# rasoolims/ImageTranslate

Hardware: AMD Instinct MI355X
Metric: train tokens/sec (whole node), 6L enc-dec d=512 seq128 b64, 1/2/4/8 GPU (higher is better)
Workload: dtype bf16; 1 GPU; 6L/6L enc-dec d=512 h=8 ff=2048 V=30000, src[64,128] tgt[64,128], synthetic random-token MT; global_batch=64, seq_len=128, parallelism=dp1, distinct_batches=8, directions=2

## Files before the change

imagetranslate_amd/csrc/gemm_ln.hip:

```cpp
#include "mma.hpp"

namespace {

constexpr int LN_BM = 32, LN_THREADS = 512, LN_RB = 128;
constexpr int LN_A_TILE = LN_BM * LN_RB;

struct GemmLnP {
  const void* A; int64_t lda; int64_t a_bytes;
  const void* W; int64_t ldw; int64_t w_bytes;
  const void* bias; const void* resid; int64_t ldr;
  const void* gamma; const void* beta;
  void* pre_ln; void* out; int64_t ldo;
  float* mean; float* rstd;
  int M, K, rotate, has_bias, has_resid;
  float eps, inv_keep; uint32_t drop_thresh; uint64_t seed;
  unsigned long long* trace;
};

template <int N> IMT_DEVICE void wait_vmcnt() { asm volatile("s_waitcnt vmcnt(%0)" ::"n"(N) : "memory"); }

template <typename T, int NTW, int SPLIT> struct LnDma {
  static constexpr int NTS = NTW / SPLIT;
  static constexpr int WP = 2 * NTS;
  __amdgpu_buffer_rsrc_t ra, rw;
  int voff_w[WP], voff_a, hstep;
  IMT_DEVICE void init(const GemmLnP& p, int m0, int wave) {
    constexpr int ES = sizeof(T);
    ra = __builtin_amdgcn_make_buffer_rsrc(const_cast<void*>(p.A), 0, (int)p.a_bytes, 0x00020000);
    rw = __builtin_amdgcn_make_buffer_rsrc(const_cast<void*>(p.W), 0, (int)p.w_bytes, 0x00020000);
    const int lane = threadIdx.x & 63, prow = lane >> 3, pc = lane & 7;
#pragma unroll
    for (int i = 0; i < WP; ++i) {
      const int lr = wave * 16 * NTS + 8 * i + prow;
      const int n = wave * 16 * NTW + 8 * i + prow;
      voff_w[i] = (int)(((int64_t)n * p.ldw) * ES + ((pc ^ swz<LN_RB>(lr)) << 4));
    }
    hstep = (int)((int64_t)16 * NTS * p.ldw * ES);
    voff_a = 0;
    if (wave < 4) {
      const int row = 8 * wave + prow;
      voff_a = (int)(((int64_t)(m0 + row) * p.lda) * ES + ((pc ^ swz<LN_RB>(row)) << 4));
    }
  }
  IMT_DEVICE void issue(char* st, int kt, int h, int wave) const {
    const int adv = kt * LN_RB;
    if (wave < 4)
      __builtin_amdgcn_raw_ptr_buffer_load_lds(ra, (__attribute__((address_space(3))) void*)(st + wave * 1024), 16, voff_a + adv, 0, 0, 0);
    const int wadv = adv + h * hstep;
#pragma unroll
    for (int i = 0; i < WP; ++i)
      __builtin_amdgcn_raw_ptr_buffer_load_lds(rw, (__attribute__((address_space(3))) void*)(st + LN_A_TILE + (wave * WP + i) * 1024), 16,
                                               voff_w[i] + wadv, 0, 0, 0);
  }
};

template <typename T, int NTW, int SPLIT, int NST>
__global__ __launch_bounds__(LN_THREADS) void gemm_ln_kernel(GemmLnP p) {
  constexpr int N = 128 * NTW, NTS = NTW / SPLIT, WP = 2 * NTS;
  constexpr int SLOT = LN_A_TILE + (N / SPLIT) * LN_RB;
  constexpr int ES = sizeof(T);
  typedef typename Frag<T>::type frag_t;
  typedef typename Vec4<T>::type raw_t;
  extern __shared__ __attribute__((aligned(16))) char smem[];
  float* red = reinterpret_cast<float*>(smem + NST * SLOT);

  const int nblk = (p.M + LN_BM - 1) / LN_BM;
  const int m0 = imt_xcd_block(blockIdx.x, nblk) * LN_BM;
  const int wave = __builtin_amdgcn_readfirstlane(threadIdx.x >> 6);
  const int lane = threadIdx.x & 63, r = lane & 15, g = lane >> 4;
  const int wn = wave * 16 * NTW;
  const int nt = (int)((int64_t)p.K * ES / LN_RB);
  const int ns = nt * SPLIT;

  LnDma<T, NTW, SPLIT> dma;
  dma.init(p, m0, wave);
  const int phase = p.rotate ? (int)((blockIdx.x >> 3) % (unsigned)nt) : 0;
  auto issue = [&](int q) {
    const int k = q / SPLIT + phase;
    dma.issue(smem + (q % NST) * SLOT, k >= nt ? k - nt : k, q % SPLIT, wave);
  };

  const T* bias = reinterpret_cast<const T*>(p.bias);
  const T* resid = reinterpret_cast<const T*>(p.resid);
  const T* gamma = reinterpret_cast<const T*>(p.gamma);
  const T* beta = reinterpret_cast<const T*>(p.beta);
  raw_t rres[2][NTW], rb[NTW], rg[NTW], rbe[NTW];
#pragma unroll
  for (int j = 0; j < NTW; ++j) {
    const int n = wn + 16 * j + 4 * g;
    rb[j] = Vec4<T>::load_raw(bias + n);
    rg[j] = Vec4<T>::load_raw(gamma + n);
    rbe[j] = Vec4<T>::load_raw(beta + n);
#pragma unroll
    for (int i = 0; i < 2; ++i) {
      const int64_t m = min(m0 + 16 * i + r, p.M - 1);
      rres[i][j] = Vec4<T>::load_raw(resid + m * p.ldr + n);
    }
  }

  f32x4 acc[2][NTW];
#pragma unroll
  for (int i = 0; i < 2; ++i)
#pragma unroll
    for (int j = 0; j < NTW; ++j) acc[i][j] = f32x4{0.f, 0.f, 0.f, 0.f};

#pragma unroll
  for (int s0 = 0; s0 < NST - 1; ++s0)
    if (s0 < ns) issue(s0);
  IMT_STAMP(p.trace, 0);
  for (int q0 = 0; q0 < ns; q0 += SPLIT) {
#pragma unroll
    for (int h = 0; h < SPLIT; ++h) {
      const int q = q0 + h;
      const int newer = min(NST - 2, ns - 1 - q);
      if (wave < 4) {
        if (newer >= 2) wait_vmcnt<2 * (WP + 1)>(); else if (newer == 1) wait_vmcnt<WP + 1>(); else wait_vmcnt<0>();
      } else {
        if (newer >= 2) wait_vmcnt<2 * WP>(); else if (newer == 1) wait_vmcnt<WP>(); else wait_vmcnt<0>();
      }
      asm volatile("s_barrier" ::: "memory");
      if (q == 0) IMT_STAMP(p.trace, 1);
      if (q + NST - 1 < ns) issue(q + NST - 1);
      const char* ta = smem + (q % NST) * SLOT;
      const char* tb = ta + LN_A_TILE;
#pragma unroll
      for (int ks = 0; ks < 2; ++ks) {
        frag_t fa[2], fb[NTS];
#pragma unroll
        for (int i = 0; i < 2; ++i) fa[i] = lds_frag_kcontig<T, LN_RB>(ta, 16 * i, 4 * ks);
#pragma unroll
        for (int j = 0; j < NTS; ++j) fb[j] = lds_frag_kcontig<T, LN_RB>(tb, wave * 16 * NTS + 16 * j, 4 * ks);
#pragma unroll
        for (int i = 0; i < 2; ++i)
#pragma unroll
          for (int j = 0; j < NTS; ++j) mma16(acc[i][h * NTS + j], fb[j], fa[i]);
      }
    }
  }
  IMT_STAMP(p.trace, 2);

  float s[2] = {0.f, 0.f};
#pragma unroll
  for (int i = 0; i < 2; ++i) {
    const int64_t m = m0 + 16 * i + r;
#pragma unroll
    for (int j = 0; j < NTW; ++j) {
      const int n = wn + 16 * j + 4 * g;
      f32x4 v = acc[i][j];
      if (p.has_bias) v += Vec4<T>::cvt(rb[j]);
      if (p.drop_thresh) dropout_apply4(v, p.seed, (uint64_t)m * (uint64_t)N + (uint64_t)n, p.drop_thresh, p.inv_keep);
      if (p.has_resid) v += Vec4<T>::cvt(rres[i][j]);
#pragma unroll
      for (int e = 0; e < 4; ++e) {
        v[e] = to_f32<T>(from_f32<T>(v[e]));
        s[i] += v[e];
      }
      acc[i][j] = v;
    }
  }
#pragma unroll
  for (int i = 0; i < 2; ++i) {
    s[i] += __shfl_xor(s[i], 16, 64);
    s[i] += __shfl_xor(s[i], 32, 64);
    if (g == 0) red[wave * 32 + 16 * i + r] = s[i];
  }
  __syncthreads();
  float mean[2], rstd[2], q[2] = {0.f, 0.f};
#pragma unroll
  for (int i = 0; i < 2; ++i) {
    float t = 0.f;
#pragma unroll
    for (int w = 0; w < 8; ++w) t += red[w * 32 + 16 * i + r];
    mean[i] = t / (float)N;
#pragma unroll
    for (int j = 0; j < NTW; ++j)
#pragma unroll
      for (int e = 0; e < 4; ++e) { const float d = acc[i][j][e] - mean[i]; q[i] += d * d; }
    q[i] += __shfl_xor(q[i], 16, 64);
    q[i] += __shfl_xor(q[i], 32, 64);
    if (g == 0) red[256 + wave * 32 + 16 * i + r] = q[i];
  }
  __syncthreads();
  IMT_STAMP(p.trace, 3);
  T* pre = reinterpret_cast<T*>(p.pre_ln);
  T* out = reinterpret_cast<T*>(p.out);
#pragma unroll
  for (int i = 0; i < 2; ++i) {
    float t = 0.f;
#pragma unroll
    for (int w = 0; w < 8; ++w) t += red[256 + w * 32 + 16 * i + r];
    rstd[i] = 1.0f / sqrtf(t / (float)N + p.eps);
    const int64_t m = m0 + 16 * i + r;
    if (m < p.M) {
#pragma unroll
      for (int j = 0; j < NTW; ++j) {
        const int n = wn + 16 * j + 4 * g;
        const f32x4 gv = Vec4<T>::cvt(rg[j]), bv = Vec4<T>::cvt(rbe[j]);
        f32x4 y;
#pragma unroll
        for (int e = 0; e < 4; ++e) y[e] = (acc[i][j][e] - mean[i]) * rstd[i] * gv[e] + bv[e];
        if (pre) Vec4<T>::store(pre + m * p.ldo + n, acc[i][j]);
        Vec4<T>::store(out + m * p.ldo + n, y);
      }
      if (wave == 0 && g == 0) {
        if (p.mean) p.mean[m] = mean[i];
        if (p.rstd) p.rstd[m] = rstd[i];
      }
    }
  }
  IMT_STAMP(p.trace, 4);
}

template <typename T, int NTW, int SPLIT, int NST>
int launch_gemm_ln(const GemmLnP& p, hipStream_t st) {
  constexpr int N = 128 * NTW;
  constexpr int LDS = NST * (LN_A_TILE + (N / SPLIT) * LN_RB) + 2 * 8 * 32 * 4;
  static_assert(LDS <= 160 * 1024, "ring does not fit the CU's LDS");
  auto k = gemm_ln_kernel<T, NTW, SPLIT, NST>;
  static bool attr = false;
  if (!attr) { (void)hipFuncSetAttribute(reinterpret_cast<const void*>(k), hipFuncAttributeMaxDynamicSharedMemorySize, LDS); attr = true; }
  const char* kind = sizeof(T) == 2 ? "gemm_ln_bf16" : "gemm_ln_f32";
  if (imt_prof_enabled() && getenv("IMT_PROF_SHAPES")) kind = imt_prof_intern(kind, p.M, N, p.K);
  ImtProfScope prof(kind, 2.0 * p.M * N * p.K, ((double)p.M * p.K + (double)N * p.K + 3.0 * p.M * N) * sizeof(T), st);
  const int blocks = imt_cdiv(p.M, LN_BM);
  ImtTrace tr("gemm_ln", blocks, st);
  GemmLnP pt = p;
  pt.trace = tr.dev;
  hipLaunchKernelGGL(k, dim3(blocks), dim3(LN_THREADS), LDS, st, pt);
  if (tr.dev) fprintf(stderr, "[gemm_ln %s %dx%dx%d]\n", kind, p.M, N, p.K);
  IMT_CHECK_LAUNCH();
  return IMT_OK;
}

}

extern "C" int imt_gemm_bias_residual_ln_supported(int dtype, int N, int K) {
  const int es = imt_dtype_bytes(dtype);
  return imt_ok_dtype(dtype) && N >= 128 && N <= 512 && N % 128 == 0 && K > 0 && ((int64_t)K * es) % LN_RB == 0;
}

extern "C" int imt_gemm_bias_residual_ln(int dtype, const void* x, int64_t ldx, const void* w, int64_t ldw, const void* bias,
                                         const void* resid, int64_t ldr, const void* gamma, const void* beta, void* pre_ln,
                                         void* out, int64_t ldo, float* mean, float* rstd, int M, int N, int K, float eps,
                                         float dropout_p, uint64_t dropout_seed, void* stream) {
  IMT_CHECK_ARG(imt_ok_dtype(dtype), "gemm_bias_residual_ln: bad dtype");
  IMT_CHECK_ARG(imt_gemm_bias_residual_ln_supported(dtype, N, K), "gemm_bias_residual_ln: N must be 128, 256, 384 or 512 and K a whole number of 128-byte tiles (N=%d K=%d)", N, K);
  if (M <= 0) return IMT_OK;
  const int es = imt_dtype_bytes(dtype), al = 16 / es;
  IMT_CHECK_ARG(x && w && gamma && beta && out, "gemm_bias_residual_ln: null pointer");
  IMT_CHECK_ARG(ldx % al == 0 && ldw % al == 0 && ldo % 4 == 0 && (!resid || ldr % 4 == 0), "gemm_bias_residual_ln: leading dimensions must keep rows 16-byte aligned");
  IMT_CHECK_ARG((((uintptr_t)x | (uintptr_t)w) & 15) == 0, "gemm_bias_residual_ln: x / w must be 16-byte aligned");
  IMT_CHECK_ARG(dropout_p >= 0.f && dropout_p < 1.f, "gemm_bias_residual_ln: dropout_p outside [0, 1)");
  GemmLnP p;
  p.A = x; p.lda = ldx; p.a_bytes = ((int64_t)(M - 1) * ldx + K) * es;
  p.W = w; p.ldw = ldw; p.w_bytes = ((int64_t)(N - 1) * ldw + K) * es;
  IMT_CHECK_ARG(p.a_bytes < (1ll << 31) && p.w_bytes < (1ll << 31), "gemm_bias_residual_ln: operand too large for 32-bit offsets");
  p.bias = bias ? bias : gamma; p.resid = resid ? resid : gamma; p.ldr = resid ? ldr : 0; p.gamma = gamma; p.beta = beta;
  p.has_bias = bias != nullptr; p.has_resid = resid != nullptr;
  p.pre_ln = pre_ln; p.out = out; p.ldo = ldo; p.mean = mean; p.rstd = rstd;
  p.M = M; p.K = K; p.eps = eps;
  static const bool no_rotate = getenv("IMT_GEMM_LN_NO_ROTATE") != nullptr;
  p.rotate = no_rotate ? 0 : 1;
  p.drop_thresh = dropout_thresh(dropout_p);
  p.inv_keep = dropout_p > 0.f ? 1.0f / (1.0f - dropout_p) : 1.0f;
  p.seed = dropout_seed;
  p.trace = nullptr;
  hipStream_t st = (hipStream_t)stream;
#define IMT_GLN(T)                                            \
  switch (N / 128) {                                          \
    case 1: return launch_gemm_ln<T, 1, 1, 4>(p, st);         \
    case 2: return launch_gemm_ln<T, 2, 1, 4>(p, st);         \
    case 3: return launch_gemm_ln<T, 3, 1, 3>(p, st);         \
    default: return launch_gemm_ln<T, 4, 2, 4>(p, st);        \
  }
  if (dtype == IMT_F32) { IMT_GLN(float) }
  IMT_GLN(bf16_t)
#undef IMT_GLN
}
```

imagetranslate_amd/csrc/model.hip:

```cpp
#include "common.hpp"
#include "decode_fused.hpp"

namespace {

struct Carver {
  char* base; int64_t off;
  explicit Carver(void* b) : base(reinterpret_cast<char*>(b)), off(0) {}
  void* take(int64_t bytes) {
    void* p = base ? base + off : nullptr;
    off += (bytes + 255) & ~(int64_t)255;
    return p;
  }
};

struct AttnWs {
  void* qkv;
  void* kv;
  int64_t kv_ld;
  void* ctx;
  float* lse;
  void* pre_ln;
  float* mean; float* rstd;
  void* out;
};
struct LayerWs {
  AttnWs self_attn, cross;
  void* z; void* h;
  void* pre_ln2; float* mean2; float* rstd2;
  void* out;
};
struct StackWs {
  void* emb_sum; float* emb_mean; float* emb_rstd; void* x0;
  LayerWs* layers;
  void* d_run;
  void* dpre[3]; void* ddrop[3];
  void* d_ctx;
  void* d_ff;
  void* d_qkv;
  void* d_q;
  void* d_kv;
  void* d_emb;
  struct Scratch { void* dpre[3]; void* ddrop[3]; void* d_ctx; void* d_ff; void* d_qkv; void* d_q; void* d_kv; } scr[2];
  void use_scratch(int l) {
    const Scratch& z = scr[l & 1];
    for (int i = 0; i < 3; ++i) { dpre[i] = z.dpre[i]; ddrop[i] = z.ddrop[i]; }
    d_ctx = z.d_ctx; d_ff = z.d_ff; d_qkv = z.d_qkv; d_q = z.d_q; d_kv = z.d_kv;
  }
  void* kv_all; void* d_kv_all;
  float* delta;
  float* ln_partial;
  float* ln_site(int site, int d) const { return ln_partial + (int64_t)site * IMT_LN_BWD_WS_FLOATS(d); }
  void* splitk; int64_t splitk_bytes;
  int64_t bytes;
};

constexpr int MAX_LAYERS = 64;

int64_t kv_w_off(const imt_stack_desc* m, const imt_layer_desc& p) { return p.cross_kv_w >= 0 ? p.cross_kv_w : p.cross_attn.qkv_w + (int64_t)m->d * m->d; }
int64_t kv_b_off(const imt_stack_desc* m, const imt_layer_desc& p) { return p.cross_kv_b >= 0 ? p.cross_kv_b : p.cross_attn.qkv_b + m->d; }
bool cross_kv_batched(const imt_stack_desc* m) {
  if (!m->is_decoder || m->n_layers < 2) return false;
  const int64_t d = m->d;
  for (int l = 0; l < m->n_layers; ++l) {
    const imt_layer_desc& p = m->layers[l];
    if (p.cross_attn.qkv_w < 0 || p.cross_kv_w < 0 || p.cross_kv_b < 0) return false;
    if (p.cross_kv_w != m->layers[0].cross_kv_w + (int64_t)l * 2 * d * d) return false;
    if (p.cross_kv_b != m->layers[0].cross_kv_b + (int64_t)l * 2 * d) return false;
  }
  return true;
}

void carve(const imt_stack_desc* m, int B, int T, int Tk, void* ws, StackWs& w, LayerWs* layers) {
  Carver c(ws);
  const int64_t N = (int64_t)B * T, Nk = (int64_t)B * Tk, d = m->d, ff = m->ff, es = imt_dtype_bytes(m->dtype);
  w.emb_sum = c.take(N * d * es); w.emb_mean = (float*)c.take(N * 4); w.emb_rstd = (float*)c.take(N * 4);
  w.x0 = c.take(N * d * es);
  w.layers = layers;
  const bool batched = cross_kv_batched(m);
  const int64_t L2d = (int64_t)m->n_layers * 2 * d;
  w.kv_all = w.d_kv_all = nullptr;
  if (batched) { w.kv_all = c.take(Nk * L2d * es); w.d_kv_all = c.take(Nk * L2d * es); }
  for (int l = 0; l < m->n_layers; ++l) {
    LayerWs& L = layers[l];
    AttnWs& s = L.self_attn;
    s.qkv = c.take(N * 3 * d * es); s.kv = nullptr; s.ctx = c.take(N * d * es);
    s.lse = (float*)c.take((int64_t)B * m->heads * T * 4);
    s.pre_ln = c.take(N * d * es); s.mean = (float*)c.take(N * 4); s.rstd = (float*)c.take(N * 4);
    s.out = c.take(N * d * es);
    AttnWs& x = L.cross;
    memset(&x, 0, sizeof(x));
    if (m->is_decoder && m->layers[l].cross_attn.qkv_w >= 0) {
      x.qkv = c.take(N * d * es); x.ctx = c.take(N * d * es);
      if (batched) { x.kv = w.kv_all ? (void*)((char*)w.kv_all + (int64_t)l * 2 * d * es) : nullptr; x.kv_ld = L2d; }
      else { x.kv = c.take(Nk * 2 * d * es); x.kv_ld = 2 * d; }
      x.lse = (float*)c.take((int64_t)B * m->heads * T * 4);
      x.pre_ln = c.take(N * d * es); x.mean = (float*)c.take(N * 4); x.rstd = (float*)c.take(N * 4);
      x.out = c.take(N * d * es);
    }
    L.z = c.take(N * ff * es); L.h = c.take(N * ff * es);
    L.pre_ln2 = c.take(N * d * es); L.mean2 = (float*)c.take(N * 4); L.rstd2 = (float*)c.take(N * 4);
    L.out = c.take(N * d * es);
  }
  w.d_run = c.take(N * d * es);
  for (int k = 0; k < 2; ++k) {
    StackWs::Scratch& z = w.scr[k];
    for (int i = 0; i < 3; ++i) { z.dpre[i] = c.take(N * d * es); z.ddrop[i] = c.take(N * d * es); }
    z.d_ctx = c.take(N * d * es);
    z.d_ff = c.take(N * ff * es);
    z.d_qkv = c.take(N * 3 * d * es);
    z.d_q = c.take(N * d * es);
    z.d_kv = c.take((Nk > 0 ? Nk : 1) * 2 * d * es);
  }
  w.use_scratch(0);
  w.d_emb = c.take(N * d * es);
  w.delta = (float*)c.take((int64_t)B * m->heads * T * 4);
  w.ln_partial = (float*)c.take((int64_t)(3 * m->n_layers + 1) * IMT_LN_BWD_WS_FLOATS(d) * 4);
  w.splitk_bytes = ((N + 127) / 128) * ((d + 127) / 128) <= 128 ? imt_gemm_splitk_ws_bytes() : 0;
  w.splitk = w.splitk_bytes ? c.take(w.splitk_bytes) : nullptr;
  w.bytes = c.off;
}

struct Ctx {
  const imt_stack_desc* m; hipStream_t st; int dtype; int64_t es;
  void* splitk = nullptr; int64_t splitk_bytes = 0;
  const char* P(int64_t off) const { return reinterpret_cast<const char*>(m->params) + off * es; }
  float* G(int64_t off) const { return m->grads + off; }
};

#define RC(x) do { int rc__ = (x); if (rc__ != IMT_OK) return rc__; } while (0)

int linear_fwd(const Ctx& c, const void* x, int64_t ldx, int M, int K, int64_t w_off, int64_t b_off, int N, void* y, int64_t ldy,
               const void* resid, int64_t ldr, void* aux, int aux_mode, float drop_p, uint64_t seed) {
  imt_gemm_args a;
  memset(&a, 0, sizeof(a));
  a.dtype = c.dtype; a.layout = IMT_NT; a.M = M; a.N = N; a.K = K;
  a.A = x; a.lda = ldx; a.B = c.P(w_off); a.ldb = K; a.C = y; a.ldc = ldy; a.c_dtype = c.dtype;
  a.bias = b_off >= 0 ? c.P(b_off) : nullptr;
  a.resid = resid; a.ldr = ldr; a.aux = aux; a.ldaux = N; a.aux_mode = aux_mode; a.split_k = 1; a.alpha = 1.f;
  a.dropout_p = drop_p; a.dropout_seed = seed;
  a.splitk_ws = c.splitk; a.splitk_ws_bytes = c.splitk_bytes;
  return imt_gemm(&a, c.st);
}

int linear_bwd_input(const Ctx& c, const void* dy, int64_t lddy, int M, int N, int64_t w_off, int K, void* dx, int64_t lddx,
                     const void* resid, int64_t ldr, void* aux, int aux_mode, int accumulate) {
  imt_gemm_args a;
  memset(&a, 0, sizeof(a));
  a.dtype = c.dtype; a.layout = IMT_NN; a.M = M; a.N = K; a.K = N;
  a.A = dy; a.lda = lddy; a.B = c.P(w_off); a.ldb = K; a.C = dx; a.ldc = lddx; a.c_dtype = c.dtype;
  a.resid = resid; a.ldr = ldr; a.aux = aux; a.ldaux = K; a.aux_mode = aux_mode; a.split_k = 1; a.alpha = 1.f;
  a.accumulate = accumulate;
  a.splitk_ws = c.splitk; a.splitk_ws_bytes = c.splitk_bytes;
  return imt_gemm(&a, c.st);
}

bool fuse_dense_ln(const Ctx& c, int M, int N, int K) {
  static const int mode = getenv("IMT_GEMM_LN") ? atoi(getenv("IMT_GEMM_LN")) : -1;
  if (mode == 0 || !imt_gemm_bias_residual_ln_supported(c.dtype, N, K)) return false;
  if (mode == 1) return true;
  return N <= 256 && K <= 1024;
}
int dense_resid_ln(const Ctx& c, const void* x, int64_t ldx, int M, int K, int64_t w_off, int64_t b_off, int N, const void* resid,
                   int64_t g_off, int64_t beta_off, void* pre_ln, void* out, float* mean, float* rstd, float drop_p, uint64_t seed) {
  if (fuse_dense_ln(c, M, N, K))
    return imt_gemm_bias_residual_ln(c.dtype, x, ldx, c.P(w_off), K, b_off >= 0 ? c.P(b_off) : nullptr, resid, N, c.P(g_off), c.P(beta_off),
                                     pre_ln, out, N, mean, rstd, M, N, K, c.m->ln_eps, drop_p, seed, c.st);
  imt_gemm_args a;
  memset(&a, 0, sizeof(a));
  a.dtype = c.dtype; a.layout = IMT_NT; a.M = M; a.N = N; a.K = K;
  a.A = x; a.lda = ldx; a.B = c.P(w_off); a.ldb = K; a.C = pre_ln; a.ldc = N; a.c_dtype = c.dtype;
  a.bias = b_off >= 0 ? c.P(b_off) : nullptr;
  a.resid = resid; a.ldr = N; a.aux_mode = IMT_AUX_NONE; a.split_k = 1; a.alpha = 1.f;
  a.dropout_p = drop_p; a.dropout_seed = seed;
  a.ln_gamma = c.P(g_off); a.ln_beta = c.P(beta_off); a.ln_out = out; a.ld_ln = N; a.ln_mean = mean; a.ln_rstd = rstd;
  a.ln_eps = c.m->ln_eps;
  a.splitk_ws = c.splitk; a.splitk_ws_bytes = c.splitk_bytes;
  return imt_gemm(&a, c.st);
}

struct DeferredDW {
  imt_gemm_args list[8];
  int n = 0;
  void add(const Ctx& c, const void* dy, int64_t lddy, const void* x, int64_t ldx, int M, int N, int K, int64_t w_off, int64_t b_off) {
    imt_gemm_args& a = list[n++];
    memset(&a, 0, sizeof(a));
    a.dtype = c.dtype; a.layout = IMT_TN; a.M = N; a.N = K; a.K = M;
    a.A = dy; a.lda = lddy; a.B = x; a.ldb = ldx; a.C = c.G(w_off); a.ldc = K; a.c_dtype = IMT_F32; a.alpha = 1.f;
    a.split_k = 1; a.accumulate = 1;
    a.a_colsum = b_off >= 0 ? c.G(b_off) : nullptr;
    const int tiles = imt_cdiv(N, 128) * imt_cdiv(K, 128);
    int sk = 1;
    while (sk < 8 && tiles * sk * 2 <= 256 && M / (sk * 2) >= 512) sk *= 2;
    if (M % (c.dtype == IMT_BF16 ? 64 : 32) != 0) { a.split_k = sk; a.accumulate = (sk == 1); }
  }
  int flush(hipStream_t st) {
    const int rc = n ? imt_gemm_grouped_tn(list, n, st) : IMT_OK;
    n = 0;
    return rc;
  }
};

struct SideQueue {
  hipStream_t st = nullptr;
  hipEvent_t ready[MAX_LAYERS], done[MAX_LAYERS];
  bool ok = false;
  bool init() {
    if (st) return ok;
    if (hipStreamCreateWithFlags(&st, hipStreamNonBlocking) != hipSuccess) { st = (hipStream_t)1; return ok = false; }
    for (int i = 0; i < MAX_LAYERS; ++i)
      if (hipEventCreateWithFlags(&ready[i], hipEventDisableTiming) != hipSuccess ||
          hipEventCreateWithFlags(&done[i], hipEventDisableTiming) != hipSuccess) return ok = false;
    return ok = true;
  }
};
SideQueue g_side;

uint64_t site_seed(uint64_t base, int layer, int site) { return base + 0x9E3779B97F4A7C15ull * (uint64_t)(layer * 16 + site + 1); }

struct MaskSet { const uint8_t* key; const uint8_t* query; const uint8_t* m3d; int causal; };

inline const char* offp(const void* p, int64_t elems, int64_t es) { return reinterpret_cast<const char*>(p) + elems * es; }
inline char* offp(void* p, int64_t elems, int64_t es) { return reinterpret_cast<char*>(p) + elems * es; }

imt_attn_args attn_block_args(const Ctx& c, const AttnWs& w, bool cross, int B, int T, int Tk, const MaskSet& ms, float drop_p,
                              uint64_t seed) {
  const int d = c.m->d;
  imt_attn_args a;
  memset(&a, 0, sizeof(a));
  a.dtype = c.dtype; a.B = B; a.H = c.m->heads; a.Tq = T; a.Tk = cross ? Tk : T; a.head_dim = d / c.m->heads;
  a.Q = w.qkv; a.ldq = cross ? d : 3 * d;
  if (cross) { a.K = w.kv; a.ldk = w.kv_ld; a.V = offp(w.kv, d, c.es); a.ldv = w.kv_ld; }
  else       { a.K = offp(w.qkv, d, c.es); a.ldk = 3 * d; a.V = offp(w.qkv, 2 * d, c.es); a.ldv = 3 * d; }
  a.O = w.ctx; a.ldo = d; a.lse = w.lse;
  a.key_mask = ms.key; a.query_mask = ms.query; a.mask3d = ms.m3d; a.causal = ms.causal;
  a.scale = 1.0f / sqrtf((float)a.head_dim);
  a.dropout_p = drop_p; a.dropout_seed = seed;
  return a;
}

int attn_block_fwd(const Ctx& c, const imt_attn_block& p, AttnWs& w, const void* x, int B, int T, const void* kv_src, int Tk,
                   const MaskSet& ms, bool training, uint64_t seed, int layer, int site0, int64_t kv_w = -1, int64_t kv_b = -1,
                   bool kv_ready = false) {
  const int d = c.m->d;
  const int N = B * T;
  const float hp = training ? c.m->hidden_dropout : 0.f, ap = training ? c.m->attn_dropout : 0.f;
  if (!kv_src) {
    RC(linear_fwd(c, x, d, N, d, p.qkv_w, p.qkv_b, 3 * d, w.qkv, 3 * d, nullptr, 0, nullptr, IMT_AUX_NONE, 0.f, 0));
  } else {
    const int Nk = B * Tk;
    RC(linear_fwd(c, x, d, N, d, p.qkv_w, p.qkv_b, d, w.qkv, d, nullptr, 0, nullptr, IMT_AUX_NONE, 0.f, 0));
    if (!kv_ready)
      RC(linear_fwd(c, kv_src, d, Nk, d, kv_w, kv_b, 2 * d, w.kv, w.kv_ld, nullptr, 0, nullptr, IMT_AUX_NONE, 0.f, 0));
  }
  const imt_attn_args a = attn_block_args(c, w, kv_src != nullptr, B, T, Tk, ms, ap, site_seed(seed, layer, site0));
  RC(imt_attention_fwd(&a, c.st));
  RC(dense_resid_ln(c, w.ctx, d, N, d, p.o_w, p.o_b, d, x, p.ln_g, p.ln_b, w.pre_ln, w.out, w.mean, w.rstd, hp, site_seed(seed, layer, site0 + 1)));
  return IMT_OK;
}

int attn_block_bwd(const Ctx& c, const imt_attn_block& p, AttnWs& w, StackWs& sw, DeferredDW& dw, int slot, const void* x, int B, int T,
                   const void* kv_src, int Tk, const MaskSet& ms, bool training, uint64_t seed, int layer, int site0, const void* dy,
                   void* d_kv_src, int accumulate_kv, int64_t kv_w = -1, int64_t kv_b = -1, void* d_kv_batched = nullptr) {
  const int d = c.m->d;
  const int N = B * T;
  const float hp = training ? c.m->hidden_dropout : 0.f, ap = training ? c.m->attn_dropout : 0.f;
  void* d_pre = sw.dpre[slot];
  void* d_dense = (hp > 0.f) ? sw.ddrop[slot] : d_pre;
  RC(imt_layernorm_bwd(c.dtype, dy, w.pre_ln, c.P(p.ln_g), w.mean, w.rstd, d_pre, c.G(p.ln_g), c.G(p.ln_b), N, d, 0.f, 0,
                       (hp > 0.f) ? d_dense : nullptr, hp, site_seed(seed, layer, site0 + 1), sw.ln_site(3 * layer + slot, d), c.st));
  dw.add(c, d_dense, d, w.ctx, d, N, d, d, p.o_w, p.o_b);
  imt_attn_args a = attn_block_args(c, w, kv_src != nullptr, B, T, Tk, ms, ap, site_seed(seed, layer, site0));
  const bool proj = imt_attention_bwd_proj_supported(a.dtype, a.head_dim, a.H, a.Tq, a.Tk, d, ms.m3d != nullptr);
  if (!proj) RC(linear_bwd_input(c, d_dense, d, N, d, p.o_w, d, sw.d_ctx, d, nullptr, 0, nullptr, IMT_AUX_NONE, 0));
  a.dO = proj ? nullptr : sw.d_ctx; a.lddo = d;
  a.delta = sw.delta;
  auto attn_bwd = [&]() { return proj ? imt_attention_bwd_proj(&a, d_dense, d, c.P(p.o_w), d, d, c.st) : imt_attention_bwd(&a, c.st); };
  if (!kv_src) {
    a.dQ = sw.d_qkv; a.lddq = 3 * d; a.dK = offp(sw.d_qkv, d, c.es); a.lddk = 3 * d; a.dV = offp(sw.d_qkv, 2 * d, c.es); a.lddv = 3 * d;
    RC(attn_bwd());
    dw.add(c, sw.d_qkv, 3 * d, x, d, N, 3 * d, d, p.qkv_w, p.qkv_b);
    RC(linear_bwd_input(c, sw.d_qkv, 3 * d, N, 3 * d, p.qkv_w, d, sw.d_run, d, d_pre, d, nullptr, IMT_AUX_NONE, 0));
  } else {
    const int Nk = B * Tk;
    void* dkv = d_kv_batched ? d_kv_batched : sw.d_kv;
    const int64_t lddkv = d_kv_batched ? w.kv_ld : 2 * d;
    a.dQ = sw.d_q; a.lddq = d; a.dK = dkv; a.lddk = lddkv; a.dV = offp(dkv, d, c.es); a.lddv = lddkv;
    RC(attn_bwd());
    dw.add(c, sw.d_q, d, x, d, N, d, d, p.qkv_w, p.qkv_b);
    RC(linear_bwd_input(c, sw.d_q, d, N, d, p.qkv_w, d, sw.d_run, d, d_pre, d, nullptr, IMT_AUX_NONE, 0));
    dw.add(c, dkv, lddkv, kv_src, d, Nk, 2 * d, d, kv_w, kv_b);
    if (!d_kv_batched) {
      if (d_kv_src)
        RC(linear_bwd_input(c, sw.d_kv, 2 * d, Nk, 2 * d, kv_w, d, d_kv_src, d, nullptr, 0, nullptr, IMT_AUX_NONE, accumulate_kv));
    }
  }
  return IMT_OK;
}

int ffn_fwd(const Ctx& c, const imt_layer_desc& p, LayerWs& w, const void* x, int N, bool training, uint64_t seed, int layer) {
  const int d = c.m->d, ff = c.m->ff;
  const float hp = training ? c.m->hidden_dropout : 0.f;
  RC(linear_fwd(c, x, d, N, d, p.ff1_w, p.ff1_b, ff, w.h, ff, nullptr, 0, w.z, IMT_AUX_GELU_FWD, 0.f, 0));
  RC(dense_resid_ln(c, w.h, ff, N, ff, p.ff2_w, p.ff2_b, d, x, p.ln2_g, p.ln2_b, w.pre_ln2, w.out, w.mean2, w.rstd2, hp, site_seed(seed, layer, 8)));
  return IMT_OK;
}

int ffn_bwd(const Ctx& c, const imt_layer_desc& p, LayerWs& w, StackWs& sw, DeferredDW& dw, const void* x, int N, bool training,
            uint64_t seed, int layer, const void* dy) {
  const int d = c.m->d, ff = c.m->ff;
  const float hp = training ? c.m->hidden_dropout : 0.f;
  void* d_pre = sw.dpre[0];
  void* d_dense = (hp > 0.f) ? sw.ddrop[0] : d_pre;
  RC(imt_layernorm_bwd(c.dtype, dy, w.pre_ln2, c.P(p.ln2_g), w.mean2, w.rstd2, d_pre, c.G(p.ln2_g), c.G(p.ln2_b), N, d, 0.f, 0,
                       (hp > 0.f) ? d_dense : nullptr, hp, site_seed(seed, layer, 8), sw.ln_site(3 * layer, d), c.st));
  dw.add(c, d_dense, d, w.h, ff, N, d, ff, p.ff2_w, p.ff2_b);
  RC(linear_bwd_input(c, d_dense, d, N, d, p.ff2_w, ff, sw.d_ff, ff, nullptr, 0, w.z, IMT_AUX_DGELU, 0));
  dw.add(c, sw.d_ff, ff, x, d, N, ff, d, p.ff1_w, p.ff1_b);
  RC(linear_bwd_input(c, sw.d_ff, ff, N, ff, p.ff1_w, d, sw.d_run, d, d_pre, d, nullptr, IMT_AUX_NONE, 0));
  return IMT_OK;
}

int validate(const imt_stack_desc* m, const imt_stack_io* io, const void* ws, int64_t ws_bytes, StackWs& w, LayerWs* layers) {
  IMT_CHECK_ARG(m && io, "stack: null descriptor");
  IMT_CHECK_ARG(imt_ok_dtype(m->dtype), "stack: bad dtype");
  IMT_CHECK_ARG(m->n_layers >= 0 && m->n_layers <= MAX_LAYERS && (m->n_layers == 0 || m->layers), "stack: bad layer table");
  IMT_CHECK_ARG(m->d > 0 && m->heads > 0 && m->d % m->heads == 0, "stack: hidden size %d not a multiple of heads %d", m->d, m->heads);
  const int dh = m->d / m->heads;
  IMT_CHECK_ARG(dh == 32 || dh == 64, "stack: head_dim %d unsupported (32 or 64)", dh);
  IMT_CHECK_ARG(m->d % 8 == 0 && m->ff % 8 == 0, "stack: d and ff must be multiples of 8");
  IMT_CHECK_ARG(io->B > 0 && io->T > 0, "stack: empty batch");
  IMT_CHECK_ARG(io->T <= m->max_pos || io->pos_ids, "stack: sequence longer than max_position_embeddings");
  IMT_CHECK_ARG(m->params && io->ids && io->out, "stack: null tensor");
  if (m->is_decoder) IMT_CHECK_ARG(io->enc_states && io->Tk > 0, "stack: decoder needs encoder states");
  carve(m, io->B, io->T, m->is_decoder ? io->Tk : 0, const_cast<void*>(ws), w, layers);
  IMT_CHECK_ARG(ws && ws_bytes >= w.bytes, "stack: workspace too small (%lld < %lld)", (long long)ws_bytes, (long long)w.bytes);
  IMT_CHECK_ARG(((uintptr_t)ws & 255) == 0, "stack: workspace must be 256-B aligned");
  return IMT_OK;
}

}

extern "C" int64_t imt_stack_workspace_bytes(const imt_stack_desc* m, int B, int T, int Tk) {
  if (!m || m->n_layers > MAX_LAYERS || (m->n_layers > 0 && !m->layers)) return -1;
  StackWs w; LayerWs layers[MAX_LAYERS];
  carve(m, B, T, m->is_decoder ? Tk : 0, nullptr, w, layers);
  return w.bytes;
}

extern "C" int imt_stack_forward(const imt_stack_desc* m, const imt_stack_io* io, void* ws, int64_t ws_bytes, void* stream) {
  StackWs w; LayerWs layers[MAX_LAYERS];
  RC(validate(m, io, ws, ws_bytes, w, layers));
  Ctx c{m, (hipStream_t)stream, m->dtype, imt_dtype_bytes(m->dtype)};
  c.splitk = w.splitk; c.splitk_bytes = w.splitk_bytes;
  const int B = io->B, T = io->T, N = B * T, d = m->d;
  const bool training = io->training != 0;
  const uint64_t seed = io->dropout_seed;
  void* x0 = (m->n_layers == 0) ? io->out : w.x0;
  auto wait_site = [&](int k) {
    if (io->wait_events && k < io->n_wait_events && io->wait_events[k])
      (void)hipStreamWaitEvent(c.st, (hipEvent_t)const_cast<void*>(io->wait_events[k]), 0);
  };
  wait_site(0);
  RC(imt_embed_ln_fwd(c.dtype, io->ids, io->pos_ids, io->type_ids, c.P(m->emb_word), c.P(m->emb_pos), c.P(m->emb_type), c.P(m->emb_ln_g),
                      c.P(m->emb_ln_b), w.emb_sum, x0, w.emb_mean, w.emb_rstd, N, T, d, m->vocab, m->max_pos, m->n_types, m->ln_eps,
                      training ? m->hidden_dropout : 0.f, site_seed(seed, 1000, 0), c.st));
  const void* x = x0;
  const MaskSet self_ms{io->key_mask, io->query_mask, io->mask3d, io->causal};
  const MaskSet cross_ms{io->enc_mask, nullptr, nullptr, 0};
  const bool batched = cross_kv_batched(m);
  if (batched)
    RC(linear_fwd(c, io->enc_states, d, B * io->Tk, d, m->layers[0].cross_kv_w, m->layers[0].cross_kv_b, m->n_layers * 2 * d, w.kv_all,
                  (int64_t)m->n_layers * 2 * d, nullptr, 0, nullptr, IMT_AUX_NONE, 0.f, 0));
  for (int l = 0; l < m->n_layers; ++l) {
    const imt_layer_desc& p = m->layers[l];
    LayerWs& L = layers[l];
    wait_site(1 + l);
    RC(attn_block_fwd(c, p.self_attn, L.self_attn, x, B, T, nullptr, 0, self_ms, training, seed, l, 0));
    const void* a = L.self_attn.out;
    if (m->is_decoder && p.cross_attn.qkv_w >= 0) {
      RC(attn_block_fwd(c, p.cross_attn, L.cross, a, B, T, io->enc_states, io->Tk, cross_ms, training, seed, l, 4, kv_w_off(m, p),
                        kv_b_off(m, p), batched));
      a = L.cross.out;
    }
    if (l == m->n_layers - 1) L.out = io->out;
    RC(ffn_fwd(c, p, L, a, N, training, seed, l));
    x = L.out;
  }
  return IMT_OK;
}

extern "C" int imt_stack_backward(const imt_stack_desc* m, const imt_stack_io* io, void* ws, int64_t ws_bytes, int layer_lo,
                                  int layer_hi, void* stream) {
  StackWs w; LayerWs layers[MAX_LAYERS];
  RC(validate(m, io, ws, ws_bytes, w, layers));
  IMT_CHECK_ARG(m->grads && io->d_out, "stack_backward: grads / d_out missing");
  IMT_CHECK_ARG(0 <= layer_lo && layer_lo <= layer_hi && layer_hi <= m->n_layers, "stack_backward: bad layer range");
  Ctx c{m, (hipStream_t)stream, m->dtype, imt_dtype_bytes(m->dtype)};
  c.splitk = w.splitk; c.splitk_bytes = w.splitk_bytes;
  const int B = io->B, T = io->T, N = B * T, d = m->d;
  const bool training = io->training != 0;
  const uint64_t seed = io->dropout_seed;
  const MaskSet self_ms{io->key_mask, io->query_mask, io->mask3d, io->causal};
  const MaskSet cross_ms{io->enc_mask, nullptr, nullptr, 0};
  const void* dy = (layer_hi == m->n_layers) ? io->d_out : w.d_run;
  const bool batched = cross_kv_batched(m);
  DeferredDW dw;
  const int64_t lnf = IMT_LN_BWD_WS_FLOATS(d);
  if (layer_hi > layer_lo) (void)hipMemsetAsync(w.ln_site(3 * layer_lo, d), 0, (size_t)(3 * (layer_hi - layer_lo)) * lnf * 4, c.st);
  if (layer_lo == 0) (void)hipMemsetAsync(w.ln_site(3 * m->n_layers, d), 0, (size_t)lnf * 4, c.st);
  static const bool side_env = !(getenv("IMT_DW_SIDE_STREAM") && atoi(getenv("IMT_DW_SIDE_STREAM")) == 0);
  const bool side = side_env && !imt_prof_enabled() && layer_lo == 0 && layer_hi == m->n_layers && m->n_layers >= 2 && g_side.init();
  int last_side = -1;
  for (int l = layer_hi - 1; l >= layer_lo; --l) {
    const imt_layer_desc& p = m->layers[l];
    LayerWs& L = layers[l];
    w.use_scratch(l);
    if (side && l + 2 < layer_hi) (void)hipStreamWaitEvent(c.st, g_side.done[l + 2], 0);
    if (l == m->n_layers - 1) L.out = io->out;
    const bool has_cross = m->is_decoder && p.cross_attn.qkv_w >= 0;
    const void* x_in = (l == 0) ? w.x0 : (const void*)layers[l - 1].out;
    const void* a_self = L.self_attn.out;
    const void* a_ffn_in = has_cross ? L.cross.out : a_self;
    RC(ffn_bwd(c, p, L, w, dw, a_ffn_in, N, training, seed, l, dy));
    if (has_cross) {
      const bool first_cross = (l == m->n_layers - 1);
      void* dkv_l = batched ? offp(w.d_kv_all, (int64_t)l * 2 * d, c.es) : nullptr;
      RC(attn_block_bwd(c, p.cross_attn, L.cross, w, dw, 1, a_self, B, T, io->enc_states, io->Tk, cross_ms, training, seed, l, 4, w.d_run,
                        io->d_enc_states, first_cross ? 0 : 1, kv_w_off(m, p), kv_b_off(m, p), dkv_l));
    }
    RC(attn_block_bwd(c, p.self_attn, L.self_attn, w, dw, 2, x_in, B, T, nullptr, 0, self_ms, training, seed, l, 0, w.d_run, nullptr, 0));
    if (side) {
      (void)hipEventRecord(g_side.ready[l], c.st);
      (void)hipStreamWaitEvent(g_side.st, g_side.ready[l], 0);
      RC(dw.flush(g_side.st));
      (void)hipEventRecord(g_side.done[l], g_side.st);
      last_side = l;
    } else {
      RC(dw.flush(c.st));
    }
    dy = w.d_run;
  }
  if (layer_lo == 0 && batched) {
    const int Nk = B * io->Tk;
    const int L2d = m->n_layers * 2 * d;
    if (io->d_enc_states)
      RC(linear_bwd_input(c, w.d_kv_all, L2d, Nk, L2d, m->layers[0].cross_kv_w, d, io->d_enc_states, d, nullptr, 0, nullptr, IMT_AUX_NONE, 0));
  }
  if (layer_lo == 0) {
    const void* dy0 = (m->n_layers == 0) ? io->d_out : dy;
    RC(imt_layernorm_bwd(c.dtype, dy0, w.emb_sum, c.P(m->emb_ln_g), w.emb_mean, w.emb_rstd, w.d_emb, c.G(m->emb_ln_g), c.G(m->emb_ln_b), N, d,
                         training ? m->hidden_dropout : 0.f, site_seed(seed, 1000, 0), nullptr, 0.f, 0, w.ln_site(3 * m->n_layers, d), c.st));
    RC(imt_embed_bwd(c.dtype, io->ids, io->pos_ids, io->type_ids, w.d_emb, c.G(m->emb_word), c.G(m->emb_pos), c.G(m->emb_type), N, T, d,
                     m->pad_id, c.st));
  }
  {
    static int64_t g_off[3 * MAX_LAYERS + 1], b_off[3 * MAX_LAYERS + 1];
    const int first = 3 * layer_lo, emb = 3 * m->n_layers;
    const int last = (layer_lo == 0) ? emb + 1 : 3 * layer_hi;
    for (int sidx = first; sidx < last; ++sidx) {
      g_off[sidx - first] = -1; b_off[sidx - first] = -1;
      if (sidx == emb) { g_off[sidx - first] = m->emb_ln_g; b_off[sidx - first] = m->emb_ln_b; continue; }
      const int l = sidx / 3, slot = sidx % 3;
// ... 194 lines not shown
```

Before: 1.140 million tokens/s.

## Specialize gemm+LN kernel waves into dedicated loader and compute roles

Reworks the fused GEMM+bias+residual+LayerNorm kernel so waves 4-7 only issue the buffer-to-LDS loads and waves 0-3 only run the MFMA loop. Each compute wave now covers twice the columns. After the main loop the second M-tile accumulator is passed to the loader waves through a free ring slot, so all 8 waves share the LayerNorm epilogue. This is meant to take the vmcnt waits and load issue off the MFMA path, at the cost of halving the number of math waves and adding an LDS hand-over. Tile and pipeline-depth choices per N are also retuned, and a new env mode widens when the fused path is used.

```diff
diff --git a/imagetranslate_amd/csrc/gemm_ln.hip b/imagetranslate_amd/csrc/gemm_ln.hip
--- a/imagetranslate_amd/csrc/gemm_ln.hip
+++ b/imagetranslate_amd/csrc/gemm_ln.hip
@@ -4,6 +4,7 @@
 
 constexpr int LN_BM = 32, LN_THREADS = 512, LN_RB = 128;
 constexpr int LN_A_TILE = LN_BM * LN_RB;
+constexpr int LN_RED_BYTES = 2 * 8 * 32 * 4;
 
 struct GemmLnP {
   const void* A; int64_t lda; int64_t a_bytes;
@@ -19,46 +20,52 @@
 
 template <int N> IMT_DEVICE void wait_vmcnt() { asm volatile("s_waitcnt vmcnt(%0)" ::"n"(N) : "memory"); }
 
-template <typename T, int NTW, int SPLIT> struct LnDma {
-  static constexpr int NTS = NTW / SPLIT;
+template <typename T, int NTC, int SPLIT> struct LnDma {
+  static constexpr int NTS = NTC / SPLIT;
   static constexpr int WP = 2 * NTS;
   __amdgpu_buffer_rsrc_t ra, rw;
   int voff_w[WP], voff_a, hstep;
-  IMT_DEVICE void init(const GemmLnP& p, int m0, int wave) {
+  IMT_DEVICE void init(const GemmLnP& p, int m0, int lw) {
     constexpr int ES = sizeof(T);
     ra = __builtin_amdgcn_make_buffer_rsrc(const_cast<void*>(p.A), 0, (int)p.a_bytes, 0x00020000);
     rw = __builtin_amdgcn_make_buffer_rsrc(const_cast<void*>(p.W), 0, (int)p.w_bytes, 0x00020000);
     const int lane = threadIdx.x & 63, prow = lane >> 3, pc = lane & 7;
 #pragma unroll
     for (int i = 0; i < WP; ++i) {
-      const int lr = wave * 16 * NTS + 8 * i + prow;
-      const int n = wave * 16 * NTW + 8 * i + prow;
+      const int lr = lw * 16 * NTS + 8 * i + prow;
+      const int n = lw * 16 * NTC + 8 * i + prow;
       voff_w[i] = (int)(((int64_t)n * p.ldw) * ES + ((pc ^ swz<LN_RB>(lr)) << 4));
     }
     hstep = (int)((int64_t)16 * NTS * p.ldw * ES);
-    voff_a = 0;
-    if (wave < 4) {
-      const int row = 8 * wave + prow;
-      voff_a = (int)(((int64_t)(m0 + row) * p.lda) * ES + ((pc ^ swz<LN_RB>(row)) << 4));
-    }
-  }
-  IMT_DEVICE void issue(char* st, int kt, int h, int wave) const {
+    const int row = 8 * lw + prow;
+    voff_a = (int)(((int64_t)(m0 + row) * p.lda) * ES + ((pc ^ swz<LN_RB>(row)) << 4));
+  }
+  IMT_DEVICE void issue(char* st, int kt, int h, int lw) const {
     const int adv = kt * LN_RB;
-    if (wave < 4)
-      __builtin_amdgcn_raw_ptr_buffer_load_lds(ra, (__attribute__((address_space(3))) void*)(st + wave * 1024), 16, voff_a + adv, 0, 0, 0);
+    __builtin_amdgcn_raw_ptr_buffer_load_lds(ra, (__attribute__((address_space(3))) void*)(st + lw * 1024), 16, voff_a + adv, 0, 0, 0);
     const int wadv = adv + h * hstep;
 #pragma unroll
     for (int i = 0; i < WP; ++i)
-      __builtin_amdgcn_raw_ptr_buffer_load_lds(rw, (__attribute__((address_space(3))) void*)(st + LN_A_TILE + (wave * WP + i) * 1024), 16,
+      __builtin_amdgcn_raw_ptr_buffer_load_lds(rw, (__attribute__((address_space(3))) void*)(st + LN_A_TILE + (lw * WP + i) * 1024), 16,
                                                voff_w[i] + wadv, 0, 0, 0);
   }
 };
 
-template <typename T, int NTW, int SPLIT, int NST>
+template <int PPS, int NST> IMT_DEVICE void wait_slots_in_flight(int newer) {
+  static_assert((NST - 2) * PPS < 64, "vmcnt is a 6-bit counter");
+  if (NST >= 5 && newer >= 3)      wait_vmcnt<3 * PPS>();
+  else if (NST >= 4 && newer >= 2) wait_vmcnt<2 * PPS>();
+  else if (newer >= 1)             wait_vmcnt<PPS>();
+  else                             wait_vmcnt<0>();
+}
+
+template <typename T, int NTC, int SPLIT, int NST>
 __global__ __launch_bounds__(LN_THREADS) void gemm_ln_kernel(GemmLnP p) {
-  constexpr int N = 128 * NTW, NTS = NTW / SPLIT, WP = 2 * NTS;
+  constexpr int N = 64 * NTC, NTS = NTC / SPLIT, WP = 2 * NTS;
   constexpr int SLOT = LN_A_TILE + (N / SPLIT) * LN_RB;
   constexpr int ES = sizeof(T);
+  static_assert(NTC % SPLIT == 0 && NTC % 2 == 0 && NST >= 3, "slot geometry");
+  static_assert(4 * NTC * 64 * 16 <= SLOT, "the accumulator hand-over of m tile 1 must fit one ring slot");
   typedef typename Frag<T>::type frag_t;
   typedef typename Vec4<T>::type raw_t;
   extern __shared__ __attribute__((aligned(16))) char smem[];
@@ -67,156 +74,178 @@
   const int nblk = (p.M + LN_BM - 1) / LN_BM;
   const int m0 = imt_xcd_block(blockIdx.x, nblk) * LN_BM;
   const int wave = __builtin_amdgcn_readfirstlane(threadIdx.x >> 6);
+  const bool loader = wave >= 4;
+  const int c = wave & 3;
+  const int mi = wave >> 2;
   const int lane = threadIdx.x & 63, r = lane & 15, g = lane >> 4;
-  const int wn = wave * 16 * NTW;
+  const int wn = c * 16 * NTC;
   const int nt = (int)((int64_t)p.K * ES / LN_RB);
   const int ns = nt * SPLIT;
 
-  LnDma<T, NTW, SPLIT> dma;
-  dma.init(p, m0, wave);
   const int phase = p.rotate ? (int)((blockIdx.x >> 3) % (unsigned)nt) : 0;
+  LnDma<T, NTC, SPLIT> dma;
   auto issue = [&](int q) {
     const int k = q / SPLIT + phase;
-    dma.issue(smem + (q % NST) * SLOT, k >= nt ? k - nt : k, q % SPLIT, wave);
+    dma.issue(smem + (q % NST) * SLOT, k >= nt ? k - nt : k, q % SPLIT, c);
   };
+  if (loader) {
+    dma.init(p, m0, c);
+    issue(0);
+  }
 
   const T* bias = reinterpret_cast<const T*>(p.bias);
   const T* resid = reinterpret_cast<const T*>(p.resid);
   const T* gamma = reinterpret_cast<const T*>(p.gamma);
   const T* beta = reinterpret_cast<const T*>(p.beta);
-  raw_t rres[2][NTW], rb[NTW], rg[NTW], rbe[NTW];
-#pragma unroll
-  for (int j = 0; j < NTW; ++j) {
+  raw_t rres[NTC], rb[NTC], rg[NTC], rbe[NTC];
+  {
+    const int64_t mr = min(m0 + 16 * mi + r, p.M - 1);
+#pragma unroll
+    for (int j = 0; j < NTC; ++j) {
+      const int n = wn + 16 * j + 4 * g;
+      rb[j] = Vec4<T>::load_raw(bias + n);
+      rg[j] = Vec4<T>::load_raw(gamma + n);
+      rbe[j] = Vec4<T>::load_raw(beta + n);
+      rres[j] = Vec4<T>::load_raw(resid + mr * p.ldr + n);
+    }
+  }
+
+  f32x4* xfer = reinterpret_cast<f32x4*>(smem + (ns % NST) * SLOT) + c * NTC * 64 + lane;
+  f32x4 v[NTC];
+
+  if (loader) {
+    constexpr int LN_RAMP = 2;
+    static_assert(LN_RAMP <= NST - 1, "ramp");
+#pragma unroll
+    for (int s0 = 1; s0 < LN_RAMP; ++s0)
+      if (s0 < ns) issue(s0);
+    wait_slots_in_flight<WP + 1, NST>(min(LN_RAMP, ns) - 1);
+    asm volatile("s_barrier" ::: "memory");
+#pragma unroll
+    for (int s0 = LN_RAMP; s0 < NST; ++s0)
+      if (s0 < ns) issue(s0);
+    for (int q = 1; q < ns; ++q) {
+      wait_slots_in_flight<WP + 1, NST>(min(NST - 2, ns - 1 - q));
+      asm volatile("s_barrier" ::: "memory");
+      if (q + NST - 1 < ns) issue(q + NST - 1);
+    }
+  } else {
+    f32x4 acc[2][NTC];
+#pragma unroll
+    for (int i = 0; i < 2; ++i)
+#pragma unroll
+      for (int j = 0; j < NTC; ++j) acc[i][j] = f32x4{0.f, 0.f, 0.f, 0.f};
+    IMT_STAMP(p.trace, 0);
+    int cur = 0;
+    for (int q0 = 0; q0 < ns; q0 += SPLIT) {
+#pragma unroll
+      for (int h = 0; h < SPLIT; ++h) {
+        asm volatile("s_waitcnt lgkmcnt(0)\n\ts_barrier" ::: "memory");
+        if (q0 + h == 0) IMT_STAMP(p.trace, 1);
+        const char* ta = smem + cur * SLOT;
+        const char* tb = ta + LN_A_TILE;
+#pragma unroll
+        for (int ks = 0; ks < 2; ++ks) {
+          frag_t fa[2], fb[NTS];
+#pragma unroll
+          for (int i = 0; i < 2; ++i) fa[i] = lds_frag_kcontig<T, LN_RB>(ta, 16 * i, 4 * ks);
+#pragma unroll
+          for (int j = 0; j < NTS; ++j) fb[j] = lds_frag_kcontig<T, LN_RB>(tb, c * 16 * NTS + 16 * j, 4 * ks);
+#pragma unroll
+          for (int i = 0; i < 2; ++i)
+#pragma unroll
+            for (int j = 0; j < NTS; ++j) mma16(acc[i][h * NTS + j], fb[j], fa[i]);
+        }
+        cur = (cur + 1 == NST) ? 0 : cur + 1;
+      }
+    }
+    IMT_STAMP(p.trace, 2);
+#pragma unroll
+    for (int j = 0; j < NTC; ++j) { xfer[j * 64] = acc[1][j]; v[j] = acc[0][j]; }
+  }
+  __syncthreads();
+  if (loader) {
+#pragma unroll
+    for (int j = 0; j < NTC; ++j) v[j] = xfer[j * 64];
+  }
+
+  const int64_t m = m0 + 16 * mi + r;
+  const int row = 16 * mi + r;
+  float s[2] = {0.f, 0.f};
+#pragma unroll
+  for (int j = 0; j < NTC; ++j) {
     const int n = wn + 16 * j + 4 * g;
-    rb[j] = Vec4<T>::load_raw(bias + n);
-    rg[j] = Vec4<T>::load_raw(gamma + n);
-    rbe[j] = Vec4<T>::load_raw(beta + n);
-#pragma unroll
-    for (int i = 0; i < 2; ++i) {
-      const int64_t m = min(m0 + 16 * i + r, p.M - 1);
-      rres[i][j] = Vec4<T>::load_raw(resid + m * p.ldr + n);
-    }
-  }
-
-  f32x4 acc[2][NTW];
-#pragma unroll
-  for (int i = 0; i < 2; ++i)
-#pragma unroll
-    for (int j = 0; j < NTW; ++j) acc[i][j] = f32x4{0.f, 0.f, 0.f, 0.f};
-
-#pragma unroll
-  for (int s0 = 0; s0 < NST - 1; ++s0)
-    if (s0 < ns) issue(s0);
-  IMT_STAMP(p.trace, 0);
-  for (int q0 = 0; q0 < ns; q0 += SPLIT) {
-#pragma unroll
-    for (int h = 0; h < SPLIT; ++h) {
-      const int q = q0 + h;
-      const int newer = min(NST - 2, ns - 1 - q);
-      if (wave < 4) {
-        if (newer >= 2) wait_vmcnt<2 * (WP + 1)>(); else if (newer == 1) wait_vmcnt<WP + 1>(); else wait_vmcnt<0>();
-      } else {
-        if (newer >= 2) wait_vmcnt<2 * WP>(); else if (newer == 1) wait_vmcnt<WP>(); else wait_vmcnt<0>();
-      }
-      asm volatile("s_barrier" ::: "memory");
-      if (q == 0) IMT_STAMP(p.trace, 1);
-      if (q + NST - 1 < ns) issue(q + NST - 1);
-      const char* ta = smem + (q % NST) * SLOT;
-      const char* tb = ta + LN_A_TILE;
-#pragma unroll
-      for (int ks = 0; ks < 2; ++ks) {
-        frag_t fa[2], fb[NTS];
-#pragma unroll
-        for (int i = 0; i < 2; ++i) fa[i] = lds_frag_kcontig<T, LN_RB>(ta, 16 * i, 4 * ks);
-#pragma unroll
-        for (int j = 0; j < NTS; ++j) fb[j] = lds_frag_kcontig<T, LN_RB>(tb, wave * 16 * NTS + 16 * j, 4 * ks);
-#pragma unroll
-        for (int i = 0; i < 2; ++i)
-#pragma unroll
-          for (int j = 0; j < NTS; ++j) mma16(acc[i][h * NTS + j], fb[j], fa[i]);
-      }
-    }
-  }
-  IMT_STAMP(p.trace, 2);
-
-  float s[2] = {0.f, 0.f};
-#pragma unroll
-  for (int i = 0; i < 2; ++i) {
-    const int64_t m = m0 + 16 * i + r;
-#pragma unroll
-    for (int j = 0; j < NTW; ++j) {
-      const int n = wn + 16 * j + 4 * g;
-      f32x4 v = acc[i][j];
-      if (p.has_bias) v += Vec4<T>::cvt(rb[j]);
-      if (p.drop_thresh) dropout_apply4(v, p.seed, (uint64_t)m * (uint64_t)N + (uint64_t)n, p.drop_thresh, p.inv_keep);
-      if (p.has_resid) v += Vec4<T>::cvt(rres[i][j]);
-#pragma unroll
-      for (int e = 0; e < 4; ++e) {
-        v[e] = to_f32<T>(from_f32<T>(v[e]));
-        s[i] += v[e];
-      }
-      acc[i][j] = v;
-    }
-  }
-#pragma unroll
-  for (int i = 0; i < 2; ++i) {
-    s[i] += __shfl_xor(s[i], 16, 64);
-    s[i] += __shfl_xor(s[i], 32, 64);
-    if (g == 0) red[wave * 32 + 16 * i + r] = s[i];
+    f32x4 x = v[j];
+    if (p.has_bias) x += Vec4<T>::cvt(rb[j]);
+    if (p.drop_thresh) dropout_apply4(x, p.seed, (uint64_t)m * (uint64_t)N + (uint64_t)n, p.drop_thresh, p.inv_keep);
+    if (p.has_resid) x += Vec4<T>::cvt(rres[j]);
+#pragma unroll
+    for (int e = 0; e < 4; ++e) {
+      x[e] = to_f32<T>(from_f32<T>(x[e]));
+      s[j / (NTC / 2)] += x[e];
+    }
+    v[j] = x;
+  }
+#pragma unroll
+  for (int h = 0; h < 2; ++h) {
+    s[h] += __shfl_xor(s[h], 16, 64);
+    s[h] += __shfl_xor(s[h], 32, 64);
+    if (g == 0) red[(2 * c + h) * 32 + row] = s[h];
   }
   __syncthreads();
-  float mean[2], rstd[2], q[2] = {0.f, 0.f};
-#pragma unroll
-  for (int i = 0; i < 2; ++i) {
-    float t = 0.f;
-#pragma unroll
-    for (int w = 0; w < 8; ++w) t += red[w * 32 + 16 * i + r];
-    mean[i] = t / (float)N;
-#pragma unroll
-    for (int j = 0; j < NTW; ++j)
-#pragma unroll
-      for (int e = 0; e < 4; ++e) { const float d = acc[i][j][e] - mean[i]; q[i] += d * d; }
-    q[i] += __shfl_xor(q[i], 16, 64);
-    q[i] += __shfl_xor(q[i], 32, 64);
-    if (g == 0) red[256 + wave * 32 + 16 * i + r] = q[i];
+  float mean = 0.f, sq[2] = {0.f, 0.f};
+#pragma unroll
+  for (int w = 0; w < 8; ++w) mean += red[w * 32 + row];
+  mean = mean / (float)N;
+#pragma unroll
+  for (int j = 0; j < NTC; ++j)
+#pragma unroll
+    for (int e = 0; e < 4; ++e) {
+      const float d = v[j][e] - mean;
+      float& q = sq[j / (NTC / 2)];
+      if (j % (NTC / 2) == 0 && e == 0) continue;
+      if (j % (NTC / 2) == 0 && e == 1) { const float d0 = v[j][0] - mean; q = __builtin_fmaf(d0, d0, __fmul_rn(d, d)); continue; }
+      q = __builtin_fmaf(d, d, q);
+    }
+#pragma unroll
+  for (int h = 0; h < 2; ++h) {
+    sq[h] += __shfl_xor(sq[h], 16, 64);
+    sq[h] += __shfl_xor(sq[h], 32, 64);
+    if (g == 0) red[256 + (2 * c + h) * 32 + row] = sq[h];
   }
   __syncthreads();
   IMT_STAMP(p.trace, 3);
   T* pre = reinterpret_cast<T*>(p.pre_ln);
   T* out = reinterpret_cast<T*>(p.out);
-#pragma unroll
-  for (int i = 0; i < 2; ++i) {
-    float t = 0.f;
-#pragma unroll
-    for (int w = 0; w < 8; ++w) t += red[256 + w * 32 + 16 * i + r];
-    rstd[i] = 1.0f / sqrtf(t / (float)N + p.eps);
-    const int64_t m = m0 + 16 * i + r;
-    if (m < p.M) {
-#pragma unroll
-      for (int j = 0; j < NTW; ++j) {
-        const int n = wn + 16 * j + 4 * g;
-        const f32x4 gv = Vec4<T>::cvt(rg[j]), bv = Vec4<T>::cvt(rbe[j]);
-        f32x4 y;
-#pragma unroll
-        for (int e = 0; e < 4; ++e) y[e] = (acc[i][j][e] - mean[i]) * rstd[i] * gv[e] + bv[e];
-        if (pre) Vec4<T>::store(pre + m * p.ldo + n, acc[i][j]);
-        Vec4<T>::store(out + m * p.ldo + n, y);
-      }
-      if (wave == 0 && g == 0) {
-        if (p.mean) p.mean[m] = mean[i];
-        if (p.rstd) p.rstd[m] = rstd[i];
-      }
+  float var = 0.f;
+#pragma unroll
+  for (int w = 0; w < 8; ++w) var += red[256 + w * 32 + row];
+  const float rstd = 1.0f / sqrtf(var / (float)N + p.eps);
+  if (m < p.M) {
+#pragma unroll
+    for (int j = 0; j < NTC; ++j) {
+      const int n = wn + 16 * j + 4 * g;
+      const f32x4 gv = Vec4<T>::cvt(rg[j]), bv = Vec4<T>::cvt(rbe[j]);
+      f32x4 y;
+#pragma unroll
+      for (int e = 0; e < 4; ++e) y[e] = (v[j][e] - mean) * rstd * gv[e] + bv[e];
+      if (pre) Vec4<T>::store(pre + m * p.ldo + n, v[j]);
+      Vec4<T>::store(out + m * p.ldo + n, y);
+    }
+    if (c == 0 && g == 0) {
+      if (p.mean) p.mean[m] = mean;
+      if (p.rstd) p.rstd[m] = rstd;
     }
   }
   IMT_STAMP(p.trace, 4);
 }
 
-template <typename T, int NTW, int SPLIT, int NST>
+template <typename T, int NTC, int SPLIT, int NST>
 int launch_gemm_ln(const GemmLnP& p, hipStream_t st) {
-  constexpr int N = 128 * NTW;
-  constexpr int LDS = NST * (LN_A_TILE + (N / SPLIT) * LN_RB) + 2 * 8 * 32 * 4;
+  constexpr int N = 64 * NTC;
+  constexpr int LDS = NST * (LN_A_TILE + (N / SPLIT) * LN_RB) + LN_RED_BYTES;
   static_assert(LDS <= 160 * 1024, "ring does not fit the CU's LDS");
-  auto k = gemm_ln_kernel<T, NTW, SPLIT, NST>;
+  auto k = gemm_ln_kernel<T, NTC, SPLIT, NST>;
   static bool attr = false;
   if (!attr) { (void)hipFuncSetAttribute(reinterpret_cast<const void*>(k), hipFuncAttributeMaxDynamicSharedMemorySize, LDS); attr = true; }
   const char* kind = sizeof(T) == 2 ? "gemm_ln_bf16" : "gemm_ln_f32";
@@ -259,8 +288,7 @@
   p.has_bias = bias != nullptr; p.has_resid = resid != nullptr;
   p.pre_ln = pre_ln; p.out = out; p.ldo = ldo; p.mean = mean; p.rstd = rstd;
   p.M = M; p.K = K; p.eps = eps;
-  static const bool no_rotate = getenv("IMT_GEMM_LN_NO_ROTATE") != nullptr;
-  p.rotate = no_rotate ? 0 : 1;
+  p.rotate = getenv("IMT_GEMM_LN_NO_ROTATE") ? 0 : 1;
   p.drop_thresh = dropout_thresh(dropout_p);
   p.inv_keep = dropout_p > 0.f ? 1.0f / (1.0f - dropout_p) : 1.0f;
   p.seed = dropout_seed;
@@ -268,10 +296,10 @@
   hipStream_t st = (hipStream_t)stream;
 #define IMT_GLN(T)                                            \
   switch (N / 128) {                                          \
-    case 1: return launch_gemm_ln<T, 1, 1, 4>(p, st);         \
-    case 2: return launch_gemm_ln<T, 2, 1, 4>(p, st);         \
-    case 3: return launch_gemm_ln<T, 3, 1, 3>(p, st);         \
-    default: return launch_gemm_ln<T, 4, 2, 4>(p, st);        \
+    case 1: return launch_gemm_ln<T, 2, 1, 4>(p, st);         \
+    case 2: return launch_gemm_ln<T, 4, 1, 4>(p, st);         \
+    case 3: return launch_gemm_ln<T, 6, 2, 5>(p, st);         \
+    default: return launch_gemm_ln<T, 8, 2, 4>(p, st);        \
   }
   if (dtype == IMT_F32) { IMT_GLN(float) }
   IMT_GLN(bf16_t)
diff --git a/imagetranslate_amd/csrc/model.hip b/imagetranslate_amd/csrc/model.hip
--- a/imagetranslate_amd/csrc/model.hip
+++ b/imagetranslate_amd/csrc/model.hip
@@ -158,6 +158,7 @@
   static const int mode = getenv("IMT_GEMM_LN") ? atoi(getenv("IMT_GEMM_LN")) : -1;
   if (mode == 0 || !imt_gemm_bias_residual_ln_supported(c.dtype, N, K)) return false;
   if (mode == 1) return true;
+  if (mode == 2 || mode == 3) return (N <= 256 && K <= 1024) || ((K <= N) == (mode == 2));
   return N <= 256 && K <= 1024;
 }
 int dense_resid_ln(const Ctx& c, const void* x, int64_t ldx, int M, int K, int64_t w_off, int64_t b_off, int N, const void* resid,
```

After: 1.140 million tokens/s, median of 4. No clear change (+0.0%).
